# fgnt/pb_bss

Measured on AMD Instinct MI355X. Metric: cACGMM EM iterations/sec on F=513,T=500,D=8,K=3, higher is better.
Workload: dtype f64; 1 GPU; BASELINE configs[1]: 8-mic 3-source cACGMM, F=513 T=500 D=8 K=3, complex64 STFT resident in HBM, fit_predict; utterances=1

## Files before the change

pb_bss_amd/csrc/cacgmm_em.hpp:

```cpp
#pragma once
#include "pbbss.h"
#include "wave_la.hpp"
#include "embed_dev.hpp"

namespace pbbss {

struct EmArgs {
  const void* y;
  int64_t B;
  int T;
  const double* gamma0;
  const double* q0;
  const double* in_eigvec;
  const double* in_eigval;
  const double* in_weight;
  int64_t wb, wk, wt;
  const double* saliency;
  const uint8_t* activity;
  const uint8_t* final_activity;
  double* out_eigvec;
  double* out_eigval;
  double* out_weight;
  int32_t* out_status;
  double* out_aff;
  double* out_q;
  double* out_logpdf;
  double* out_cov;
  char* scratch;
  size_t scratch_stride;
  unsigned long long* prof;
  int T_total;
  int split_groups;
  int split_window;
  int64_t b_first;
  double* xslab;
  unsigned* xcount;
  int* xerror;
  int xepoch;
  int split_prio;
  int main_grid;
  unsigned lds_given;
  unsigned xbuf_given;
  unsigned spin_limit;
  int wgroup;
  double* gsum;
  double* gaff;
  double* gw;
  unsigned* gcount;
  double* out_weight_shared;
  int iterations;
  int covariance_norm;
  int weight_mode;
  int layout;
  int final_predict;
  int force_eig;
  double aff_eps;
  double final_eps;
  double eig_floor;
};

struct JointExtras {
  const double* extra_logpdf;
  double spatial_weight;
  const int* perm;
  const double* state_in;
  double* state_out;
  int emit_model;
  double* weight_fk_out;
  int main_grid;
  unsigned lds_given;
  unsigned xbuf_given;
};

struct JointMs {
  int mode;
  double* q_out;
  double* lndet_out;
  double* weight_fk_out;
  unsigned lds_given;
  int main_grid;
  SpectralFin fin;
};

template <int D, int K, typename YS, bool SPILL = false>
struct EmKernel {
  static constexpr int DP = (D + 1) / 2;
  static constexpr int NOFF = D * (D - 1) / 2;
  static constexpr int NA = D * D;
  static constexpr int NDW = (D + kEmWaves - 1) / kEmWaves;
  static constexpr int NOW = (NOFF + kEmWaves - 1) / kEmWaves;
#ifndef PBBSS_E_CHUNK
#define PBBSS_E_CHUNK 1
#endif
#ifndef PBBSS_E_PAIR
#define PBBSS_E_PAIR 0
#endif
#ifndef PBBSS_M_PREFETCH
#define PBBSS_M_PREFETCH 0
#endif
  static constexpr int kOperandChunk = PBBSS_E_CHUNK;
  using YS4 = typename std::conditional<std::is_same<YS, float>::value, float4, double4>::type;
  using YS2 = typename std::conditional<std::is_same<YS, float>::value, float2, double2>::type;

  struct Lds {
    YS* ybuf;
    double* inv_n2;
    double* wbuf;
    double* cpack;
    double* apack;
    double* wgt;
    double* detm;
    double* rdet;
    double* red;
    double* ssum;
    int* dete;
    int* status;
    int* flags;
    unsigned short* wbtab;
    double* sink;
    int Tp;
  };

  static constexpr int kFC = 64;
  static __host__ __device__ __forceinline__ int padded_frames(int T) { return (T + kFC - 1) & ~(kFC - 1); }
  static __host__ __device__ __forceinline__ int yoff(int dp, int t) {
    return ((((t >> 6) * DP + dp) << 6) + (t & 63)) * 4;
  }
  static __host__ __device__ __forceinline__ int woff(int k, int t) {
    return (((t >> 6) * K + k) << 6) + (t & 63);
  }
  static __host__ __device__ size_t frame_bytes(int T) {
    size_t Tp = (size_t)padded_frames(T);
    return (size_t)DP * Tp * 4 * sizeof(YS) + Tp * 8 + (size_t)K * Tp * 8;
  }
  static __host__ __device__ size_t small_bytes() {
    size_t n = 0;
    n += (size_t)K * NA * 8;
    n += (size_t)K * NA * 8;
    n += (size_t)K * 8 * 4;
    n += (size_t)kEmWaves * K * 8;
    n += (size_t)K * 4 * 2 + 16;
    n += wbtab_bytes() + 8;
    return n;
  }
  static __host__ __device__ size_t lds_bytes(int T) {
    size_t n = small_bytes() + (SPILL ? 0 : frame_bytes(T));
    return (n + 15) & ~(size_t)15;
  }
  static __host__ __device__ size_t scratch_bytes(int T) {
    return SPILL ? ((frame_bytes(T) + 255) & ~(size_t)255) : 0;
  }

  static __device__ Lds carve_small(char* p, int Tp) {
    Lds L;
    L.Tp = Tp;
    L.ybuf = nullptr;
    L.inv_n2 = nullptr;
    L.wbuf = nullptr;
    carve_small_into(L, p);
    return L;
  }

  static __device__ Lds carve(char* base, int T, char* scratch = nullptr) {
    Lds L;
    L.Tp = padded_frames(T);
    char* p = base;
    char* f = SPILL ? scratch : base;
    L.ybuf = reinterpret_cast<YS*>(f);
    f += (size_t)DP * L.Tp * 4 * sizeof(YS);
    L.inv_n2 = reinterpret_cast<double*>(f);
    f += (size_t)L.Tp * 8;
    L.wbuf = reinterpret_cast<double*>(f);
    f += (size_t)K * L.Tp * 8;
    if (!SPILL) p = f;
    carve_small_into(L, p);
    fill_wbtab(L);
    return L;
  }

  static __device__ __forceinline__ void carve_small_into(Lds& L, char* p) {
    L.cpack = reinterpret_cast<double*>(p);
    p += (size_t)K * NA * 8;
    L.apack = reinterpret_cast<double*>(p);
    p += (size_t)K * NA * 8;
    L.wgt = reinterpret_cast<double*>(p);
    p += K * 8;
    L.detm = reinterpret_cast<double*>(p);
    p += K * 8;
    L.rdet = reinterpret_cast<double*>(p);
    p += K * 8;
    L.ssum = reinterpret_cast<double*>(p);
    p += K * 8;
    L.red = reinterpret_cast<double*>(p);
    p += kEmWaves * K * 8;
    L.dete = reinterpret_cast<int*>(p);
    p += K * 4;
    L.status = reinterpret_cast<int*>(p);
    p += K * 4;
    L.flags = reinterpret_cast<int*>(p);
    p += 16;
    L.wbtab = reinterpret_cast<unsigned short*>(p);
    p += wbtab_bytes();
    L.sink = reinterpret_cast<double*>(p);
  }

  static __device__ __forceinline__ int t_stride(const EmArgs& a) {
    return a.T_total ? a.T_total : a.T;
  }

  static __device__ __forceinline__ void load_frame(const Lds& L, int t, double (&re)[D],
                                                    double (&im)[D]) {
    PBBSS_DEV_ASSERT(t >= 0 && t < L.Tp);
    static_for<0, DP>([&](auto dpc) {
      constexpr int dp = dpc;
      YS4 v = *reinterpret_cast<const YS4*>(L.ybuf + yoff(dp, t));
      re[2 * dp] = (double)v.x;
      im[2 * dp] = (double)v.y;
      if constexpr (2 * dp + 1 < D) {
        re[2 * dp + 1] = (double)v.z;
        im[2 * dp + 1] = (double)v.w;
      }
    });
  }

  static __device__ void phase_load(const EmArgs& a, const Lds& L, int64_t b, int tid,
                                    int tf = 0) {
    const int T = a.T;
    const int TS = t_stride(a);
    const YS2* yg = reinterpret_cast<const YS2*>(a.y);
    bool zero_seen = false;
    for (int t = tid; t < L.Tp; t += kEmThreads) {
      double n2 = 0.0;
      YS vr[2 * DP], vi[2 * DP];
#pragma unroll
      for (int d = 0; d < 2 * DP; ++d) {
        vr[d] = (YS)0;
        vi[d] = (YS)0;
      }
      if (t < T) {
#pragma unroll
        for (int d = 0; d < D; ++d) {
          size_t idx = (a.layout == PBBSS_LAYOUT_TD) ? ((size_t)b * TS + tf + t) * D + d
                                                     : ((size_t)b * D + d) * TS + tf + t;
          YS2 v = yg[idx];
          vr[d] = v.x;
          vi[d] = v.y;
          n2 += (double)v.x * (double)v.x + (double)v.y * (double)v.y;
        }
      }
#pragma unroll
      for (int dp = 0; dp < DP; ++dp) {
        YS4 o;
        o.x = vr[2 * dp];
        o.y = vi[2 * dp];
        o.z = vr[2 * dp + 1];
        o.w = vi[2 * dp + 1];
        *reinterpret_cast<YS4*>(L.ybuf + yoff(dp, t)) = o;
      }
      double inv;
      if (a.layout == PBBSS_LAYOUT_TD) {
        inv = (n2 > 0.0) ? 1.0 / n2 : 0.0;
      } else {
        inv = 1.0;
      }
      L.inv_n2[t] = (t < T) ? inv : 0.0;
      if (t < T && !(n2 > 0.0)) zero_seen = true;
      if (t >= T) {
#pragma unroll
        for (int k = 0; k < K; ++k) L.wbuf[woff(k, t)] = 0.0;
      }
    }
    if (zero_seen) atomicOr(L.flags, 1);
  }

  static __device__ __forceinline__ double mweight(double g_sal, double q, double inv_n2) {
    return g_sal / fmax(q, 10.0 * kTiny) * inv_n2;
  }

  static __device__ void phase_init_gamma(const EmArgs& a, const Lds& L, int64_t b, int tid,
                                          int wave, int lane, int tf = 0) {
    const int TS = t_stride(a);
    double s[K];
#pragma unroll
    for (int k = 0; k < K; ++k) s[k] = 0.0;
    for (int t = tid; t < a.T; t += kEmThreads) {
      double sal = a.saliency ? a.saliency[(size_t)b * TS + tf + t] : 1.0;
      double inv = L.inv_n2[t];
#pragma unroll
      for (int k = 0; k < K; ++k) {
        size_t idx = ((size_t)b * K + k) * TS + tf + t;
        double g = a.gamma0[idx] * sal;
        double q = a.q0 ? a.q0[idx] : 1.0;
        L.wbuf[woff(k, t)] = mweight(g, q, inv);
        if (a.gaff && a.weight_mode == PBBSS_WEIGHT_SHARED_KT)
          __hip_atomic_store(a.gaff + idx, g, __ATOMIC_RELAXED, __HIP_MEMORY_SCOPE_AGENT);
        s[k] += g;
      }
    }
#pragma unroll
    for (int k = 0; k < K; ++k) {
      double tot = wave_sum(s[k]);
      if (lane == 0) L.red[wave * K + k] = tot;
    }
  }

  template <bool FINAL, bool TW, bool JOINT = false, bool PAIR = false, bool PERM = false>
  static __device__ void phase_e(const EmArgs& a, const Lds& L, int64_t b, int tid, int wave,
                                 int lane, double eps, int tf = 0,
                                 const JointExtras* jx = nullptr,
                                 const double* w_kt = nullptr,
                                 double* pub_kt = nullptr) {
    tid = opaque(tid);
    lane = opaque(lane);
    const int TS = t_stride(a);
    static_assert(!JOINT || !PAIR, "joint E-step is written for one frame per lane");
    double s[K];
#pragma unroll
    for (int k = 0; k < K; ++k) s[k] = 0.0;
    double jlogdet[K];
#pragma unroll
    for (int k = 0; k < K; ++k)
      jlogdet[k] = JOINT ? log(L.detm[k]) + (double)L.dete[k] * 0.6931471805599453 : 0.0;
    auto pass = [&](int t0, auto nfc) {
      constexpr int NF = decltype(nfc)::value;
      if (t0 + wave * kWave >= padded_frames(a.T)) return;
      int tl[NF];
      int tt[NF];
      bool ok[NF];
      bool inl[NF];
      double re[NF][D], im[NF][D], q[NF][K];
#pragma unroll
      for (int f = 0; f < NF; ++f) {
        int t = t0 + f * kEmThreads + tid;
        ok[f] = t < a.T;
        inl[f] = (f == 0) || t < padded_frames(a.T);
        tt[f] = ok[f] ? t : (a.T - 1);
        tl[f] = (f == 0) ? t : min(t, padded_frames(a.T) - 1);
        load_frame(L, tl[f], re[f], im[f]);
#pragma unroll
        for (int k = 0; k < K; ++k) q[f][k] = 0.0;
      }
      {
        constexpr int NG = (NA + 15) / 16;
        double areg[K][NG];
#pragma unroll
        for (int k = 0; k < K; ++k) {
#pragma unroll
          for (int g = 0; g < NG; ++g) {
            const int e = 16 * g + (lane & 15);
            areg[k][g] = L.apack[k * NA + (e < NA ? e : NA - 1)];
          }
        }
        static_for<0, D>([&](auto ic) {
// ... 128 lines not shown
          double qq = fmax(fabs(q[f][k] * inv), kTiny);
          q[f][k] = qq;
          int e;
          double m = frexp(qq, &e);
          double rm = fast_rcp(m);
          rq[k] = ldexp(rm, -e);
          val[k] = rdet[k] * ipow<D>(rm);
          ex[k] = -(e * D + dete[k]);
          emax = max(emax, ex[k]);
        }
        double g[K], den = 0.0;
#pragma unroll
        for (int k = 0; k < K; ++k) {
          double w;
          if constexpr (TW) {
            w = w_kt ? __hip_atomic_load(w_kt + (size_t)k * TS + tf + t, __ATOMIC_RELAXED,
                                         __HIP_MEMORY_SCOPE_AGENT)
                     : a.in_weight[b * a.wb + k * a.wk + (int64_t)(tf + t) * a.wt];
          } else {
            w = wgt[k];
          }
          double v = ldexp(val[k], ex[k] - emax) * w;
          const uint8_t* act = FINAL ? a.final_activity : a.activity;
          if (act) v *= (double)act[((size_t)b * K + k) * TS + tf + t];
          g[k] = v;
          den += v;
        }
        const double poison = den - den;
        den = fmax(den, kTiny);
        const double rden = fast_rcp(den);
        const double sal = (!FINAL && a.saliency) ? a.saliency[(size_t)b * TS + tf + t] : 1.0;
        const double invp = inv + poison;
#pragma unroll
        for (int k = 0; k < K; ++k) {
          double gam = g[k] * rden;
          if (!FINAL || eps != 0.0) gam = fmin(fmax(gam, eps), 1.0 - eps);
          if constexpr (FINAL) {
            gam += poison;
            if (ok[f]) {
              size_t idx = ((size_t)b * K + k) * TS + tf + t;
              if (a.out_aff) a.out_aff[idx] = gam;
              if (a.out_q) a.out_q[idx] = q[f][k];
              if (a.out_logpdf) {
                a.out_logpdf[idx] = -(double)D * log(q[f][k]) -
                                    (log(detm[k]) + (double)dete[k] * 0.6931471805599453);
              }
            }
          } else {
            double gs = ok[f] ? gam * sal : 0.0;
            if (pub_kt && ok[f])
              __hip_atomic_store(pub_kt + (size_t)k * TS + tf + t, gs, __ATOMIC_RELAXED,
                                 __HIP_MEMORY_SCOPE_AGENT);
            double rqk = fmin(rq[k], 1.0 / (10.0 * kTiny));
            if (f == 0 || inl[f]) L.wbuf[woff(k, tl[f])] = gs * rqk * invp;
            s[k] += gs;
          }
        }
      }
      }
    };
    {
      int t0 = 0;
      if constexpr (PAIR) {
        for (; a.T - t0 > kEmThreads; t0 += 2 * kEmThreads) pass(t0, std::integral_constant<int, 2>{});
      }
      for (; t0 < a.T; t0 += kEmThreads) pass(t0, std::integral_constant<int, 1>{});
    }
    if constexpr (!FINAL) wave_class_sums<K>(s, lane, L.red + wave * K);
  }

  static constexpr int NSLOT = NDW + 2 * NOW;
  static constexpr int NACC = ((K * NSLOT + 15) / 16) * 16;

  struct EntryMap {
    int dwave[D], drank[D];
    int pwave[NOFF > 0 ? NOFF : 1], prank[NOFF > 0 ? NOFF : 1];
    unsigned long long dcode[kEmWaves], pcode[kEmWaves];
  };
  static constexpr EntryMap make_entry_map() {
    EntryMap m{};
    int nd[kEmWaves] = {}, np[kEmWaves] = {};
    for (int w = 0; w < kEmWaves; ++w) {
      m.dcode[w] = ~0ull;
      m.pcode[w] = ~0ull;
    }
    for (int i = 0; i < D; ++i) {
      int w = i % kEmWaves;
      if (D == 8) w = (i < 2) ? 0 : (i < 4) ? 3 : (i < 6) ? 1 : 2;
      m.dwave[i] = w;
      m.drank[i] = nd[w]++;
    }
    for (int p = 0; p < NOFF; ++p) {
      const int i = tri_i<D>(p), j = tri_j<D>(p);
      int w = p % kEmWaves;
      if (D == 8) {
        if (j < 4) w = 0;
        else if (i >= 4) w = 1;
        else if (i == 0 && j == 4) w = 0;
        else if (i == 3 && j == 7) w = 1;
        else w = (i < 2) ? 2 : 3;
      }
      m.pwave[p] = w;
      m.prank[p] = np[w]++;
    }
    for (int i = 0; i < D; ++i) {
      const int w = m.dwave[i], r = m.drank[i];
      m.dcode[w] = (m.dcode[w] & ~(15ull << (4 * r))) | ((unsigned long long)i << (4 * r));
    }
    for (int p = 0; p < NOFF; ++p) {
      const int w = m.pwave[p], r = m.prank[p];
      m.pcode[w] = (m.pcode[w] & ~(31ull << (5 * r))) | ((unsigned long long)p << (5 * r));
    }
    return m;
  }
  static constexpr EntryMap kMap = make_entry_map();
  static constexpr bool entry_map_fits() {
    for (int i = 0; i < D; ++i)
      if (kMap.drank[i] >= NDW) return false;
    for (int p = 0; p < NOFF; ++p)
      if (kMap.prank[p] >= NOW) return false;
    return true;
  }
  static_assert(entry_map_fits(), "a wave owns more entries than it has accumulator slots");

  static constexpr int kWbR = NACC / 16;
  static __host__ __device__ constexpr size_t wbtab_bytes() {
    return ((size_t)kEmWaves * 16 * kWbR * sizeof(unsigned short) + 7) & ~(size_t)7;
  }
  template <bool ROUND_ROBIN = false>
  static __device__ __forceinline__ void fill_wbtab(const Lds& L) {
    const int tid = threadIdx.x;
    if (tid >= kEmWaves * 16) return;
    const int w = tid >> 4, g = tid & 15;
    const unsigned long long dcode = kMap.dcode[w], pcode = kMap.pcode[w];
    const int sink = (int)(L.sink - L.cpack);
#pragma unroll
    for (int m = 0; m < kWbR; ++m) {
      const int idx = kWbR * g + m;
      int off = sink;
      if (idx < K * NSLOT) {
        const int k = idx / NSLOT, sl = idx % NSLOT;
        const bool dg = sl < NDW;
        const int u = ROUND_ROBIN
                          ? (dg ? sl * kEmWaves + w : ((sl - NDW) >> 1) * kEmWaves + w)
                          : (dg ? (int)((dcode >> (4 * sl)) & 15)
                                : (int)((pcode >> (5 * ((sl - NDW) >> 1))) & 31));
        const int e = dg ? u : D + 2 * u + ((sl - NDW) & 1);
        if (u < (dg ? D : NOFF)) off = k * NA + e;
      }
      L.wbtab[(w * 16 + g) * kWbR + m] = (unsigned short)off;
    }
  }

  template <int W>
  static __device__ void phase_m(const EmArgs& a, const Lds& L, int lane, int c_begin = 0,
                                 int c_end = -1, double* cpack_out = nullptr) {
    lane = opaque(lane);
    double acc[NACC];
    const YS* yp = L.ybuf + (size_t)lane * 4 + (size_t)c_begin * (DP * kFC * 4);
    const double* wp = L.wbuf + lane + (size_t)c_begin * (K * kFC);
    struct Raw {
      YS4 v[DP];
      double w[K];
    };
    auto fetch = [&](Raw& r) {
      static_for<0, DP>([&](auto dpc) {
        constexpr int dp = dpc;
        r.v[dp] = *reinterpret_cast<const YS4*>(yp + dp * (kFC * 4));
      });
#pragma unroll
      for (int k = 0; k < K; ++k) r.w[k] = wp[k * kFC];
      yp += DP * kFC * 4;
      wp += K * kFC;
    };
    auto compute = [&](const Raw& r, auto firstc) {
      constexpr bool FIRST = firstc;
      double re[D], im[D];
      static_for<0, DP>([&](auto dpc) {
        constexpr int dp = dpc;
        re[2 * dp] = (double)r.v[dp].x;
        im[2 * dp] = (double)r.v[dp].y;
        if constexpr (2 * dp + 1 < D) {
          re[2 * dp + 1] = (double)r.v[dp].z;
          im[2 * dp + 1] = (double)r.v[dp].w;
        }
      });
      const double (&w)[K] = r.w;
      static_for<0, D>([&](auto ic) {
        constexpr int i = ic;
        if constexpr (kMap.dwave[i] == W) {
          double dg = re[i] * re[i] + im[i] * im[i];
#pragma unroll
          for (int k = 0; k < K; ++k) {
            double& x = acc[k * NSLOT + kMap.drank[i]];
            x = FIRST ? w[k] * dg : fma(w[k], dg, x);
          }
        }
      });
      static_for<0, NOFF>([&](auto pc) {
        constexpr int p = pc;
        if constexpr (kMap.pwave[p] == W) {
          constexpr int i = tri_i<D>(p), j = tri_j<D>(p);
          constexpr int s = NDW + 2 * kMap.prank[p];
          double pr = re[i] * re[j] + im[i] * im[j];
          double pim = im[i] * re[j] - re[i] * im[j];
#pragma unroll
          for (int k = 0; k < K; ++k) {
            double& xr = acc[k * NSLOT + s];
            double& xi = acc[k * NSLOT + s + 1];
            xr = FIRST ? w[k] * pr : fma(w[k], pr, xr);
            xi = FIRST ? w[k] * pim : fma(w[k], pim, xi);
          }
        }
      });
    };
    static_for<0, NACC>([&](auto xc) {
      constexpr int x = xc;
      constexpr int sl = x % NSLOT;
      constexpr bool used =
          x < K * NSLOT &&
          (sl < NDW ? (int)((kMap.dcode[W] >> (4 * sl)) & 15) < D
                    : (int)((kMap.pcode[W] >> (5 * ((sl - NDW) >> 1))) & 31) < NOFF);
      if constexpr (!used) acc[x] = 0.0;
    });
    const int nchunk = (c_end < 0 ? (padded_frames(a.T) >> 6) : c_end) - c_begin;
#if PBBSS_M_PREFETCH
    {
      Raw A, B;
      fetch(A);
      if (nchunk > 1) {
        fetch(B);
        __builtin_amdgcn_sched_barrier(0);
        compute(A, std::true_type{});
        int c = nchunk - 1;
        while (c > 2) {
          fetch(A);
          __builtin_amdgcn_sched_barrier(0);
          compute(B, std::false_type{});
          fetch(B);
          __builtin_amdgcn_sched_barrier(0);
          compute(A, std::false_type{});
          c -= 2;
        }
        if (c == 2) {
          fetch(A);
          __builtin_amdgcn_sched_barrier(0);
          compute(B, std::false_type{});
          compute(A, std::false_type{});
        } else {
          compute(B, std::false_type{});
        }
      } else {
        compute(A, std::true_type{});
      }
    }
#else
    {
      Raw r;
      fetch(r);
      compute(r, std::true_type{});
      for (int c = nchunk; c > 1; --c) {
        fetch(r);
        compute(r, std::false_type{});
      }
    }
#endif
#ifdef PBBSS_PHASE_PROFILE
    unsigned long long tm0 = __builtin_readcyclecounter(), tm1 = tm0;
#endif
    if (a.split_groups == 0) __builtin_amdgcn_s_setprio(1);
    wave_reduce_scatter<NACC>(acc, lane);
#ifdef PBBSS_PHASE_PROFILE
    tm1 = __builtin_readcyclecounter();
#endif
    if ((lane & 3) == 0) {
      const unsigned short* tab = L.wbtab + (W * 16 + ((lane >> 2) & 15)) * kWbR;
      double* dst = cpack_out ? cpack_out : L.cpack;
#pragma unroll
      for (int m = 0; m < kWbR; ++m) dst[tab[m]] = acc[m];
    }
    if (a.split_groups == 0) __builtin_amdgcn_s_setprio(0);
#ifdef PBBSS_PHASE_PROFILE
    if (a.prof && lane == 0 && W == 0) {
      unsigned long long tm2 = __builtin_readcyclecounter();
      atomicAdd(a.prof + 64, tm1 - tm0);
      atomicAdd(a.prof + 65, tm2 - tm1);
      atomicAdd(a.prof + 66, 1ull);
    }
#endif
  }

  static __device__ __forceinline__ int pair_index(int i, int j) {
    return i * D - (i * (i + 1)) / 2 + (j - i - 1);
  }

  static __device__ __forceinline__ void cov_entry(const Lds& L, int k, int i, int j, double& re,
                                                   double& im) {
    if (i == j) {
      re = L.cpack[k * NA + i];
      im = 0.0;
    } else {
      const int lo = min(i, j), hi = max(i, j);
      const double2 v = *reinterpret_cast<const double2*>(L.cpack + k * NA + D + 2 * pair_index(lo, hi));
      re = v.x;
      im = (i < j) ? v.y : -v.y;
    }
  }

  static __device__ __forceinline__ void store_apack(const Lds& L, int k, LaneIJ c, double gre,
                                                     double gim) {
    if (c.i < D && c.j < D) {
      if (c.i == c.j) {
        L.apack[k * NA + c.i] = gre;
      } else if (c.i < c.j) {
        int p = pair_index(c.i, c.j);
        L.apack[k * NA + D + 2 * p] = 2.0 * gre;
        L.apack[k * NA + D + 2 * p + 1] = 2.0 * gim;
      }
    }
  }

  static __device__ __forceinline__ void inverse_from_eig(double vre, double vim, double lam_col,
                                                          LaneIJ c, double& gre, double& gim) {
    gre = 0.0;
    gim = 0.0;
#pragma unroll
    for (int e = 0; e < D; ++e) {
      double il = 1.0 / lane_get(lam_col, ij_lane(0, e));
      double ar = lane_get(vre, ij_lane(c.i, e)), ai = lane_get(vim, ij_lane(c.i, e));
      double br = lane_get(vre, ij_lane(c.j, e)), bi = lane_get(vim, ij_lane(c.j, e));
      gre += (ar * br + ai * bi) * il;
      gim += (ai * br - ar * bi) * il;
    }
  }

  static __device__ void factor_class(const EmArgs& a, const Lds& L, int64_t b, int k, int lane,
                                      bool last) {
    if (a.split_groups == 0) __builtin_amdgcn_s_setprio(3);
    lane = opaque(lane);
    const LaneIJ c = lane_ij(lane);
    const bool valid = c.i < D && c.j < D;
#ifdef PBBSS_PHASE_PROFILE
    unsigned long long fs[6] = {0, 0, 0, 0, 0, 0};
    int fsn = 0;
#define PBBSS_FSTAMP fs[fsn++] = __builtin_readcyclecounter();
    PBBSS_FSTAMP
#else
#define PBBSS_FSTAMP
#endif
    double are = 0.0, aim = 0.0;
    if (valid) cov_entry(L, k, c.i, c.j, are, aim);
    double S = 0.0, tot = 0.0;
#pragma unroll
    for (int kk = 0; kk < K; ++kk) {
      double sk = 0.0;
#pragma unroll
      for (int w = 0; w < kEmWaves; ++w) sk += L.red[w * K + kk];
      tot += fabs(sk);
      S = (kk == k) ? sk : S;
    }
    const double scale = (double)D * fast_rcp(fmax(S, kTiny));
    are *= scale;
    aim *= scale;
    int st = 0;
    if (last && a.out_cov && valid) {
      double* oc = a.out_cov + ((((size_t)b * K + k) * D + c.i) * D + c.j) * 2;
      oc[0] = are;
      oc[1] = aim;
    }
    bool need_eig = last || a.force_eig || (*L.flags & 1);
    PBBSS_FSTAMP
    if (!need_eig) {
      double gre = are, gim = aim;
      ScaledReal det;
      double trc = wave_sum((valid && c.i == c.j) ? are : 0.0);
      int info = wave_hpd_inverse<D>(gre, gim, c, det);
      bool ok = (info == 0);
      PBBSS_FSTAMP
      if (ok) {
        store_apack(L, k, c, gre, gim);
        if (lane == 0) {
          L.detm[k] = det.m;
          L.rdet[k] = fast_rcp(det.m);
          L.dete[k] = det.e;
        }
        double fro2 = wave_sum(valid ? gre * gre + gim * gim : 0.0);
        const double bound2 = trc * trc * fro2;
        ok = isfinite(bound2) && (bound2 * (a.eig_floor * a.eig_floor) < 1e-4) && (bound2 < 1e26);
      }
      if (!ok) {
        need_eig = true;
        st |= PBBSS_ST_SLOWPATH;
      }
      PBBSS_FSTAMP
#ifdef PBBSS_PHASE_PROFILE
      if (a.prof && lane == 0 && k == 0 && !need_eig) {
        atomicAdd(a.prof + 67, fs[1] - fs[0]);
        atomicAdd(a.prof + 68, fs[2] - fs[1]);
        atomicAdd(a.prof + 69, fs[3] - fs[2]);
        atomicAdd(a.prof + 70, 1ull);
      }
#endif
    }
    if (need_eig) {
      const bool finite_in = isfinite(are) && isfinite(aim);
      if (wave_or(finite_in ? 0 : 1)) st |= PBBSS_ST_NONFINITE;
    }
    if (need_eig) {
      if (a.covariance_norm == PBBSS_COVNORM_TRACE) {
        double tr = wave_sum((valid && c.i == c.j) ? are : 0.0);
        double it = 1.0 / fmax(tr, kTiny);
        are *= it;
        aim *= it;
      }
      double vre, vim;
      int sweeps = wave_jacobi_heev<D>(are, aim, c, vre, vim);
      if (sweeps < 0) st |= PBBSS_ST_EIG_NOCONV;
      double lam = lane_get(are, ij_lane(c.j, c.j));
      double lmax = wave_max((c.i == 0 && c.j < D) ? lam : -1.79e308);
      double lout;
      if (a.covariance_norm == PBBSS_COVNORM_EIGENVALUE) {
        lout = lam / fmax(lmax, kTiny);
        if (lout < a.eig_floor) {
          lout = a.eig_floor;
          if (c.i == 0 && c.j < D) st |= PBBSS_ST_FLOORED;
        }
      } else {
        double fl = lmax * a.eig_floor;
        lout = lam;
        if (lout < fl) {
          lout = fl;
          if (c.i == 0 && c.j < D) st |= PBBSS_ST_FLOORED;
        }
      }
      if (c.i == 0 && c.j < D && !isfinite(lout)) st |= PBBSS_ST_NONFINITE;
      st = wave_or(st);
      if (c.j >= D) lout = 1.0;
      if (last) {
        int rank = wave_sort_rank<D>(lam, c);
        if (valid) {
          if (a.out_eigvec) {
            double* ov = a.out_eigvec + ((((size_t)b * K + k) * D + c.i) * D + rank) * 2;
            ov[0] = vre;
            ov[1] = vim;
          }
          if (a.out_eigval && c.i == 0) a.out_eigval[((size_t)b * K + k) * D + rank] = lout;
        }
      }
      double gre, gim;
      inverse_from_eig(vre, vim, lout, c, gre, gim);
      store_apack(L, k, c, gre, gim);
      ScaledReal det{1.0, 0};
#pragma unroll
      for (int e = 0; e < D; ++e) scaled_mul(det, fmax(lane_get(lout, ij_lane(0, e)), kTiny));
      if (lane == 0) {
        L.detm[k] = det.m;
        L.rdet[k] = 1.0 / det.m;
        L.dete[k] = det.e;
      }
    }
    if (lane == 0) {
      L.status[k] |= st;
      double wnew;
      if (a.weight_mode >= PBBSS_WEIGHT_SHARED_K) {
        wnew = L.wgt[k];
      } else if (a.weight_mode == PBBSS_WEIGHT_UNIFORM) {
        wnew = 1.0 / K;
      } else if (a.saliency) {
        wnew = S / ((tot == 0.0) ? 1e-10 : tot);
      } else {
        wnew = S / (double)t_stride(a);
      }
      L.wgt[k] = wnew;
    }
    if (a.split_groups == 0) __builtin_amdgcn_s_setprio(0);
  }

  static __device__ void prep_from_model(const EmArgs& a, const Lds& L, int64_t b, int k,
                                         int lane) {
    const LaneIJ c = lane_ij(lane);
    const bool valid = c.i < D && c.j < D;
    double vre = 0.0, vim = 0.0, lam = 1.0;
    if (valid) {
      const double* v = a.in_eigvec + ((((size_t)b * K + k) * D + c.i) * D + c.j) * 2;
      vre = v[0];
      vim = v[1];
      lam = a.in_eigval[((size_t)b * K + k) * D + c.j];
    }
    double gre, gim;
    inverse_from_eig(vre, vim, lam, c, gre, gim);
    store_apack(L, k, c, gre, gim);
    ScaledReal det{1.0, 0};
#pragma unroll
    for (int e = 0; e < D; ++e) scaled_mul(det, fmax(lane_get(lam, ij_lane(0, e)), kTiny));
    if (lane == 0) {
      L.detm[k] = det.m;
      L.rdet[k] = 1.0 / det.m;
      L.dete[k] = det.e;
      L.wgt[k] = a.in_weight ? a.in_weight[b * a.wb + k * a.wk] : 1.0 / K;
    }
  }

  static __device__ __forceinline__ void quad_forms(const Lds& L, int t, double (&q)[K]) {
    double re[D], im[D];
    load_frame(L, t, re, im);
#pragma unroll
    for (int k = 0; k < K; ++k) q[k] = 0.0;
    static_for<0, D>([&](auto ic) {
      constexpr int i = ic;
      double dg = re[i] * re[i] + im[i] * im[i];
#pragma unroll
      for (int k = 0; k < K; ++k) q[k] = fma(L.apack[k * NA + i], dg, q[k]);
    });
    static_for<0, NOFF>([&](auto pc) {
      constexpr int p = pc;
      constexpr int i = tri_i<D>(p), j = tri_j<D>(p);
      double pr = re[i] * re[j] + im[i] * im[j];
      double pim = im[i] * re[j] - re[i] * im[j];
#pragma unroll
      for (int k = 0; k < K; ++k)
        q[k] = fma(L.apack[k * NA + D + 2 * p], pr, fma(L.apack[k * NA + D + 2 * p + 1], pim, q[k]));
    });
    const double inv = L.inv_n2[t];
#pragma unroll
    for (int k = 0; k < K; ++k) q[k] = fmax(fabs(q[k] * inv), kTiny);
  }

  static __device__ __forceinline__ void quad_forms_pipelined(const Lds& L, const double (&re)[D],
                                                              const double (&im)[D],
                                                              double (&q)[K]) {
    constexpr int NCH = (NOFF + kOperandChunk - 1) / kOperandChunk;
    double op[2][kOperandChunk][K][2];
    auto fetch = [&](auto cc, auto bb) {
      constexpr int c = cc, bsel = bb;
#pragma unroll
      for (int x = 0; x < kOperandChunk; ++x) {
        if (c * kOperandChunk + x < NOFF) {
#pragma unroll
          for (int k = 0; k < K; ++k) {
            op[bsel][x][k][0] = L.apack[k * NA + D + 2 * (c * kOperandChunk + x)];
            op[bsel][x][k][1] = L.apack[k * NA + D + 2 * (c * kOperandChunk + x) + 1];
          }
        }
      }
    };
#pragma unroll
    for (int k = 0; k < K; ++k) q[k] = 0.0;
    if constexpr (NCH > 0) fetch(std::integral_constant<int, 0>{}, std::integral_constant<int, 0>{});
    asm volatile("" ::: "memory");
    static_for<0, D>([&](auto ic) {
      constexpr int i = ic;
      double ad[K];
#pragma unroll
      for (int k = 0; k < K; ++k) ad[k] = L.apack[k * NA + i];
      double dg = re[i] * re[i] + im[i] * im[i];
#pragma unroll
      for (int k = 0; k < K; ++k) q[k] = fma(ad[k], dg, q[k]);
    });
    static_for<0, NCH>([&](auto cc) {
      constexpr int c = cc;
      constexpr int cur = c & 1;
      if constexpr (c + 1 < NCH) {
        fetch(std::integral_constant<int, c + 1>{}, std::integral_constant<int, 1 - cur>{});
      }
      asm volatile("" ::: "memory");
      __builtin_amdgcn_sched_barrier(0);
      static_for<0, kOperandChunk>([&](auto xc) {
        constexpr int x = xc;
        constexpr int p = c * kOperandChunk + x;
        if constexpr (p < NOFF) {
          constexpr int i = tri_i<D>(p), j = tri_j<D>(p);
          double pr = re[i] * re[j] + im[i] * im[j];
          double pim = im[i] * re[j] - re[i] * im[j];
#pragma unroll
          for (int k = 0; k < K; ++k)
            q[k] = fma(op[cur][x][k][0], pr, fma(op[cur][x][k][1], pim, q[k]));
        }
      });
#pragma unroll
      for (int k = 0; k < K; ++k) asm volatile("" : "+v"(q[k])::"memory");
      __builtin_amdgcn_sched_barrier(0);
    });
  }

  static __device__ __forceinline__ void nth_permutation(int p, int (&perm)[K]) {
    int fact = 1;
#pragma unroll
    for (int i = 2; i < K; ++i) fact *= i;
    unsigned used = 0;
#pragma unroll
    for (int i = 0; i < K; ++i) {
      int d = p / fact;
      p -= d * fact;
      if (i < K - 1) fact /= (K - 1 - i);
      int pick = 0;
#pragma unroll
      for (int c = 0, seen = 0; c < K; ++c) {
        if (!(used >> c & 1)) {
          if (seen == d) pick = c;
          ++seen;
        }
      }
      used |= 1u << pick;
      perm[i] = pick;
    }
  }

  static __device__ void phase_joint_pa(const EmArgs& a, const Lds& L, int64_t b, int tid,
                                        int wave, int lane, const JointExtras& jx, int* perm_out) {
    for (int t = tid; t < a.T; t += kEmThreads) {
      double q[K];
      quad_forms(L, t, q);
#pragma unroll
      for (int k = 0; k < K; ++k) {
// ... 815 lines not shown
          tk[k] = 0.0;
#pragma unroll
          for (int w = 0; w < kEmWaves; ++w) tk[k] += tmp[(w * K + k) * kSliceFrames + tid];
          norm += fabs(tk[k]);
        }
#pragma unroll
        for (int k = 0; k < K; ++k) {
          const double w = a.saliency ? tk[k] / ((norm == 0.0) ? 1e-10 : norm)
                                      : tk[k] / (double)a.wgroup;
          __hip_atomic_store(dst + (size_t)k * TS + t, w, __ATOMIC_RELAXED,
                             __HIP_MEMORY_SCOPE_AGENT);
        }
        asm volatile("s_waitcnt vmcnt(0)" ::: "memory");
      }
      __syncthreads();
      if (tid == 0)
        __hip_atomic_fetch_add(a.gcount + grp * 16 + 8, 1u, __ATOMIC_RELAXED,
                               __HIP_MEMORY_SCOPE_AGENT);
    }
  }

  static __device__ const double* shared_acquire_kt(const EmArgs& a, int64_t b, int step, int tid) {
    const int TS = t_stride(a);
    const int64_t grp = b / a.wgroup;
    const int nsl = (TS + kSliceFrames - 1) / kSliceFrames;
    if (tid == 0) shared_spin(a, a.gcount + grp * 16 + 8, (unsigned)nsl * (unsigned)(step + 1));
    __syncthreads();
    return a.gw + ((size_t)(step & 1) * (a.B / a.wgroup) + grp) * K * TS;
  }

  static __device__ void run_shared(const EmArgs& a, char* smem) {
    const int tid = threadIdx.x;
    const int wave = __builtin_amdgcn_readfirstlane(tid >> 6);
    const int lane = tid & 63;
    const Lds L = carve(smem, a.T, nullptr);
    const int64_t b = a.b_first + blockIdx.x;
    const bool kt = (a.weight_mode == PBBSS_WEIGHT_SHARED_KT);
    const int TS = t_stride(a);
    if (tid < K) L.status[tid] = 0;
    if (tid == 0) *L.flags = 0;
    __syncthreads();
    phase_load(a, L, b, tid);
    __syncthreads();
    const bool model_in = (a.gamma0 == nullptr);
    if (model_in) {
      for (int k = wave; k < K; k += kEmWaves) prep_from_model(a, L, b, k, lane);
      __syncthreads();
      if (!kt && tid < K) L.wgt[tid] = a.in_weight[(b / a.wgroup) * K + tid];
    } else {
      phase_init_gamma(a, L, b, tid, wave, lane);
    }
    if (kt) asm volatile("s_waitcnt vmcnt(0)" ::: "memory");
    __syncthreads();
    for (int it = 0; it < a.iterations; ++it) {
      if (it > 0 || model_in) {
        double* pub = kt ? a.gaff + ((size_t)(it & 1) * a.B + b) * K * TS : nullptr;
        if (kt) {
          const double* w_kt = (it == 0) ? a.in_weight + (b / a.wgroup) * (int64_t)K * TS
                                         : shared_acquire_kt(a, b, it - 1, tid);
          phase_e<false, true, false, false>(a, L, b, tid, wave, lane, a.aff_eps, 0, nullptr, w_kt,
                                             pub);
        } else {
          if (it > 0) shared_acquire_k(a, L, b, it - 1, tid, wave, lane);
          phase_e<false, false, false, PBBSS_E_PAIR != 0>(a, L, b, tid, wave, lane, a.aff_eps);
        }
        if (kt) asm volatile("s_waitcnt vmcnt(0)" ::: "memory");
        __syncthreads();
      }
      shared_post(a, L, b, it, tid);
      switch (wave) {
        case 0: phase_m<0>(a, L, lane); break;
        case 1: phase_m<1>(a, L, lane); break;
        case 2: phase_m<2>(a, L, lane); break;
        default: phase_m<3>(a, L, lane); break;
      }
      __syncthreads();
      const bool last = (it == a.iterations - 1);
      for (int k = wave; k < K; k += kEmWaves) factor_class(a, L, b, k, lane, last);
      __syncthreads();
      if (kt) shared_reduce_kt(a, L, b, it, tid, wave, lane);
    }
    const double* w_kt = nullptr;
    if (a.iterations > 0) {
      const int64_t grp = b / a.wgroup;
      if (kt) {
        w_kt = shared_acquire_kt(a, b, a.iterations - 1, tid);
        if (a.out_weight_shared && b == grp * a.wgroup) {
          for (int i = tid; i < K * TS; i += kEmThreads)
            a.out_weight_shared[(size_t)grp * K * TS + i] =
                __hip_atomic_load(w_kt + i, __ATOMIC_RELAXED, __HIP_MEMORY_SCOPE_AGENT);
        }
      } else {
        shared_acquire_k(a, L, b, a.iterations - 1, tid, wave, lane);
        if (a.out_weight_shared && b == grp * a.wgroup && tid < K)
          a.out_weight_shared[(size_t)grp * K + tid] = L.wgt[tid];
      }
    }
    if (tid < K && a.out_status) {
      int st = L.status[tid];
      if (split_failed(a))
        st |= PBBSS_ST_EIG_NOCONV | PBBSS_ST_NONFINITE;
      a.out_status[(size_t)b * K + tid] = st;
    }
    if (a.final_predict) {
      if (w_kt) {
        phase_e<true, true>(a, L, b, tid, wave, lane, a.final_eps, 0, nullptr, w_kt);
      } else {
        phase_e<true, false>(a, L, b, tid, wave, lane, a.final_eps);
      }
    }
  }

  static __device__ void run(const EmArgs& a, char* smem) {
    const int tid = threadIdx.x;
    const int wave = __builtin_amdgcn_readfirstlane(tid >> 6);
    const int lane = tid & 63;
    PBBSS_DEV_ASSERT(a.lds_given == 0 || lds_bytes(a.T) <= a.lds_given);
    const Lds L = carve(smem, a.T, SPILL ? a.scratch + (size_t)blockIdx.x * a.scratch_stride : nullptr);
#ifdef PBBSS_PHASE_PROFILE
    unsigned long long pc[8] = {0, 0, 0, 0, 0, 0, 0, 0};
    unsigned long long tprev = __builtin_readcyclecounter();
#define PBBSS_TICK(i)                                        \
  {                                                          \
    unsigned long long tn = __builtin_readcyclecounter();    \
    pc[i] += tn - tprev;                                     \
    tprev = tn;                                              \
  }
#else
#define PBBSS_TICK(i)
#endif
    for (int64_t b = blockIdx.x; b < a.B; b += gridDim.x) {
      __syncthreads();
      if (tid < K) L.status[tid] = 0;
      if (tid == 0) *L.flags = 0;
      __syncthreads();
      phase_load(a, L, b, tid);
      __syncthreads();
      const bool model_in = (a.gamma0 == nullptr);
      if (model_in) {
        for (int k = wave; k < K; k += kEmWaves) prep_from_model(a, L, b, k, lane);
      } else {
        phase_init_gamma(a, L, b, tid, wave, lane);
      }
      __syncthreads();
      PBBSS_TICK(0)
      for (int it = 0; it < a.iterations; ++it) {
        if (it > 0 || model_in) {
          phase_e<false, false, false, PBBSS_E_PAIR != 0>(a, L, b, tid, wave, lane, a.aff_eps);
          PBBSS_TICK(1)
          __syncthreads();
          PBBSS_TICK(2)
        }
        switch (wave) {
          case 0: phase_m<0>(a, L, lane); break;
          case 1: phase_m<1>(a, L, lane); break;
          case 2: phase_m<2>(a, L, lane); break;
          default: phase_m<3>(a, L, lane); break;
        }
        PBBSS_TICK(3)
        __syncthreads();
        PBBSS_TICK(4)
        const bool last = (it == a.iterations - 1);
        for (int k = wave; k < K; k += kEmWaves) factor_class(a, L, b, k, lane, last);
        PBBSS_TICK(5)
        __syncthreads();
        PBBSS_TICK(6)
      }
      if (tid < K) {
        if (a.out_weight && a.iterations > 0) a.out_weight[(size_t)b * K + tid] = L.wgt[tid];
        if (a.out_status) a.out_status[(size_t)b * K + tid] = L.status[tid];
      }
      if (a.final_predict) {
        if (a.iterations == 0 && a.wt != 0) {
          phase_e<true, true>(a, L, b, tid, wave, lane, a.final_eps);
        } else {
          phase_e<true, false>(a, L, b, tid, wave, lane, a.final_eps);
        }
      }
      PBBSS_TICK(7)
    }
#ifdef PBBSS_PHASE_PROFILE
    if (a.prof && lane == 0) {
      for (int i = 0; i < 8; ++i) atomicAdd(a.prof + wave * 8 + i, pc[i]);
    }
#endif
  }
};

#ifndef PBBSS_EM_WAVES
#define PBBSS_EM_WAVES 3
#endif
constexpr int em_waves_per_simd(int K) { return K <= 4 ? PBBSS_EM_WAVES : 2; }

template <int D, int K, typename YS, bool SPILL>
__global__ void __launch_bounds__(kEmThreads, em_waves_per_simd(K)) cacgmm_em_kernel(EmArgs a) {
  extern __shared__ __attribute__((aligned(16))) char smem[];
  EmKernel<D, K, YS, SPILL>::run(a, smem);
}


template <int D, int K, typename YS, bool PA>
__global__ void __launch_bounds__(kEmThreads, em_waves_per_simd(K))
    cacgmm_joint_kernel(EmArgs a, JointExtras jx) {
  extern __shared__ __attribute__((aligned(16))) char smem[];
  EmKernel<D, K, YS, false>::template run_joint<PA>(a, jx, smem);
}

template <int D, int K, typename YS, int MODE>
__global__ void __launch_bounds__(kEmThreads, em_waves_per_simd(K))
    cacgmm_joint_ms_kernel(EmArgs a, JointMs jm) {
  extern __shared__ __attribute__((aligned(16))) char smem[];
  EmKernel<D, K, YS, false>::template run_joint_ms<MODE>(a, jm, smem);
}

template <int D, int K, typename YS>
__global__ void __launch_bounds__(kEmThreads, em_waves_per_simd(K)) cacgmm_em_shared_kernel(EmArgs a) {
  extern __shared__ __attribute__((aligned(16))) char smem[];
  EmKernel<D, K, YS, false>::run_shared(a, smem);
}

template <int D, int K, typename YS>
__global__ void __launch_bounds__(kEmThreads, em_waves_per_simd(K)) cacgmm_em_split_kernel(EmArgs a) {
  extern __shared__ __attribute__((aligned(16))) char smem[];
  EmKernel<D, K, YS, false>::run_split(a, smem, (int)blockIdx.x, (int)gridDim.x);
}

}
```

Before: 79580 EM iterations/s (utterance-iterations, whole job).

## Hoist class scale and weight prep into M-step, table-drive factor loads/stores

Moves the per-class reduction of E-step sums (scale and new mixture weight) out of factor_class and into phase_m, computing it after the first chunk so it overlaps with the accumulation loop. An inline-asm pin keeps the compiler from sinking it. It also adds an LDS lookup table mapping each lane to its packed covariance offset and conjugation/store flags, replacing the per-lane index arithmetic in cov_entry and store_apack. This trims serial work on the critical factor path between barriers, at the cost of extra LDS, register pressure in phase_m, and duplicated logic.

```diff
diff --git a/pb_bss_amd/csrc/cacgmm_em.hpp b/pb_bss_amd/csrc/cacgmm_em.hpp
--- a/pb_bss_amd/csrc/cacgmm_em.hpp
+++ b/pb_bss_amd/csrc/cacgmm_em.hpp
@@ -112,10 +112,12 @@
     double* detm;
     double* rdet;
     double* red;
+    double* scale;
     double* ssum;
     int* dete;
     int* status;
     int* flags;
+    unsigned* ftab;
     unsigned short* wbtab;
     double* sink;
     int Tp;
@@ -139,7 +141,9 @@
     n += (size_t)K * NA * 8;
     n += (size_t)K * 8 * 4;
     n += (size_t)kEmWaves * K * 8;
+    n += (size_t)K * 8;
     n += (size_t)K * 4 * 2 + 16;
+    n += (size_t)kWave * 4;
     n += wbtab_bytes() + 8;
     return n;
   }
@@ -175,6 +179,7 @@
     if (!SPILL) p = f;
     carve_small_into(L, p);
     fill_wbtab(L);
+    fill_ftab(L);
     return L;
   }
 
@@ -193,12 +198,16 @@
     p += K * 8;
     L.red = reinterpret_cast<double*>(p);
     p += kEmWaves * K * 8;
+    L.scale = reinterpret_cast<double*>(p);
+    p += K * 8;
     L.dete = reinterpret_cast<int*>(p);
     p += K * 4;
     L.status = reinterpret_cast<int*>(p);
     p += K * 4;
     L.flags = reinterpret_cast<int*>(p);
     p += 16;
+    L.ftab = reinterpret_cast<unsigned*>(p);
+    p += kWave * 4;
     L.wbtab = reinterpret_cast<unsigned short*>(p);
     p += wbtab_bytes();
     L.sink = reinterpret_cast<double*>(p);
@@ -633,10 +642,67 @@
     }
   }
 
-  template <int W>
+  static constexpr unsigned kFtDiag = 1u << 10, kFtConj = 1u << 11, kFtValid = 1u << 12;
+  static constexpr unsigned kFtStore = 1u << 26, kFtStoreDiag = 1u << 27;
+  static __device__ __forceinline__ void fill_ftab(const Lds& L) {
+    const int tid = threadIdx.x;
+    if (tid >= kWave) return;
+    const LaneIJ c = lane_ij(tid);
+    unsigned t = 0;
+    if (c.i < D && c.j < D) {
+      if (c.i == c.j) {
+        t = (unsigned)(c.i * 8) | kFtDiag | kFtValid | ((unsigned)(c.i * 8) << 16) | kFtStore |
+            kFtStoreDiag;
+      } else {
+        const int lo = min(c.i, c.j), hi = max(c.i, c.j);
+        const unsigned off = (unsigned)(D + 2 * pair_index(lo, hi)) * 8;
+        t = off | kFtValid;
+        if (c.i < c.j) t |= (off << 16) | kFtStore;
+        else t |= kFtConj;
+      }
+    }
+    L.ftab[tid] = t;
+  }
+
+  static __device__ __forceinline__ void pinned(double& x, const double* after) {
+    asm volatile(""
+                 : "+v"(x)
+                 : "v"(after[0]), "v"(after[1]), "v"(after[2]), "v"(after[3]), "v"(after[4]),
+                   "v"(after[5]), "v"(after[6]), "v"(after[7]), "v"(after[8]), "v"(after[9]),
+                   "v"(after[10]), "v"(after[11]), "v"(after[12]), "v"(after[13]), "v"(after[14]),
+                   "v"(after[15]));
+  }
+  static __device__ __forceinline__ void class_prep(const EmArgs& a, const double (&red)[kEmWaves * K],
+                                                    int k, const double (&after)[48], double& scale,
+                                                    double& wnew) {
+    double S = 0.0, tot = 0.0;
+#pragma unroll
+    for (int kk = 0; kk < K; ++kk) {
+      double sk = 0.0;
+#pragma unroll
+      for (int w = 0; w < kEmWaves; ++w) sk += red[w * K + kk];
+      tot += fabs(sk);
+      S = (kk == k) ? sk : S;
+    }
+    scale = (double)D * fast_rcp(fmax(S, kTiny));
+    pinned(scale, after);
+    pinned(tot, after + 16);
+    const double den = a.saliency ? ((tot == 0.0) ? 1e-10 : tot) : (double)t_stride(a);
+    wnew = S / den;
+    pinned(wnew, after + 32);
+    if (a.weight_mode == PBBSS_WEIGHT_UNIFORM) wnew = 1.0 / K;
+  }
+
+  template <int W, bool PREP = false>
   static __device__ void phase_m(const EmArgs& a, const Lds& L, int lane, int c_begin = 0,
                                  int c_end = -1, double* cpack_out = nullptr) {
     lane = opaque(lane);
+    constexpr bool kPrep = PREP && W < K;
+    double red[kEmWaves * K];
+    if constexpr (kPrep) {
+#pragma unroll
+      for (int i = 0; i < kEmWaves * K; ++i) red[i] = L.red[i];
+    }
     double acc[NACC];
     const YS* yp = L.ybuf + (size_t)lane * 4 + (size_t)c_begin * (DP * kFC * 4);
     const double* wp = L.wbuf + lane + (size_t)c_begin * (K * kFC);
@@ -704,6 +770,25 @@
                     : (int)((kMap.pcode[W] >> (5 * ((sl - NDW) >> 1))) & 31) < NOFF);
       if constexpr (!used) acc[x] = 0.0;
     });
+    auto prep = [&]() {
+      if constexpr (kPrep) {
+        constexpr int kOwn = (K - W + kEmWaves - 1) / kEmWaves;
+        double scale[kOwn], wnew[kOwn];
+        double after[48];
+#pragma unroll
+        for (int i = 0; i < 48; ++i) after[i] = acc[i < K * NSLOT ? i : K * NSLOT - 1];
+#pragma unroll
+        for (int n = 0; n < kOwn; ++n)
+          class_prep(a, red, W + n * kEmWaves, after, scale[n], wnew[n]);
+        if (lane == 0) {
+#pragma unroll
+          for (int n = 0; n < kOwn; ++n) {
+            L.scale[W + n * kEmWaves] = scale[n];
+            if (a.weight_mode < PBBSS_WEIGHT_SHARED_K) L.wgt[W + n * kEmWaves] = wnew[n];
+          }
+        }
+      }
+    };
     const int nchunk = (c_end < 0 ? (padded_frames(a.T) >> 6) : c_end) - c_begin;
 #if PBBSS_M_PREFETCH
     {
@@ -713,6 +798,7 @@
         fetch(B);
         __builtin_amdgcn_sched_barrier(0);
         compute(A, std::true_type{});
+        prep();
         int c = nchunk - 1;
         while (c > 2) {
           fetch(A);
@@ -733,6 +819,7 @@
         }
       } else {
         compute(A, std::true_type{});
+        prep();
       }
     }
 #else
@@ -740,6 +827,7 @@
       Raw r;
       fetch(r);
       compute(r, std::true_type{});
+      prep();
       for (int c = nchunk; c > 1; --c) {
         fetch(r);
         compute(r, std::false_type{});
@@ -801,6 +889,17 @@
     }
   }
 
+  static __device__ __forceinline__ void store_apack_tab(const Lds& L, int k, unsigned ft,
+                                                         double gre, double gim) {
+    if (ft & kFtStore) {
+      double* dst = reinterpret_cast<double*>(reinterpret_cast<char*>(L.apack + k * NA) +
+                                              ((ft >> 16) & 0x3FFu));
+      const bool dg = (ft & kFtStoreDiag) != 0;
+      dst[0] = dg ? gre : 2.0 * gre;
+      if (!dg) dst[1] = 2.0 * gim;
+    }
+  }
+
   static __device__ __forceinline__ void inverse_from_eig(double vre, double vim, double lam_col,
                                                           LaneIJ c, double& gre, double& gim) {
     gre = 0.0;
@@ -815,6 +914,7 @@
     }
   }
 
+  template <bool HOISTED = false>
   static __device__ void factor_class(const EmArgs& a, const Lds& L, int64_t b, int k, int lane,
                                       bool last) {
     if (a.split_groups == 0) __builtin_amdgcn_s_setprio(3);
@@ -830,17 +930,28 @@
 #define PBBSS_FSTAMP
 #endif
     double are = 0.0, aim = 0.0;
-    if (valid) cov_entry(L, k, c.i, c.j, are, aim);
-    double S = 0.0, tot = 0.0;
-#pragma unroll
-    for (int kk = 0; kk < K; ++kk) {
-      double sk = 0.0;
-#pragma unroll
-      for (int w = 0; w < kEmWaves; ++w) sk += L.red[w * K + kk];
-      tot += fabs(sk);
-      S = (kk == k) ? sk : S;
-    }
-    const double scale = (double)D * fast_rcp(fmax(S, kTiny));
+    double S = 0.0, tot = 0.0, scale;
+    unsigned ft = 0;
+    if constexpr (HOISTED) {
+      ft = L.ftab[lane];
+      const double* cp = reinterpret_cast<const double*>(
+          reinterpret_cast<const char*>(L.cpack + k * NA) + (ft & 0x3FFu));
+      const double v0 = cp[0], v1 = cp[1];
+      scale = L.scale[k];
+      are = (ft & kFtValid) ? v0 : 0.0;
+      aim = (ft & kFtDiag) || !(ft & kFtValid) ? 0.0 : ((ft & kFtConj) ? -v1 : v1);
+    } else {
+      if (valid) cov_entry(L, k, c.i, c.j, are, aim);
+#pragma unroll
+      for (int kk = 0; kk < K; ++kk) {
+        double sk = 0.0;
+#pragma unroll
+        for (int w = 0; w < kEmWaves; ++w) sk += L.red[w * K + kk];
+        tot += fabs(sk);
+        S = (kk == k) ? sk : S;
+      }
+      scale = (double)D * fast_rcp(fmax(S, kTiny));
+    }
     are *= scale;
     aim *= scale;
     int st = 0;
@@ -859,11 +970,21 @@
       bool ok = (info == 0);
       PBBSS_FSTAMP
       if (ok) {
-        store_apack(L, k, c, gre, gim);
-        if (lane == 0) {
-          L.detm[k] = det.m;
-          L.rdet[k] = fast_rcp(det.m);
-          L.dete[k] = det.e;
+        if constexpr (HOISTED) {
+          const double rdet = fast_rcp(det.m);
+          store_apack_tab(L, k, ft, gre, gim);
+          if (lane == 0) {
+            L.detm[k] = det.m;
+            L.rdet[k] = rdet;
+            L.dete[k] = det.e;
+          }
+        } else {
+          store_apack(L, k, c, gre, gim);
+          if (lane == 0) {
+            L.detm[k] = det.m;
+            L.rdet[k] = fast_rcp(det.m);
+            L.dete[k] = det.e;
+          }
         }
         double fro2 = wave_sum(valid ? gre * gre + gim * gim : 0.0);
         const double bound2 = trc * trc * fro2;
@@ -930,7 +1051,8 @@
       }
       double gre, gim;
       inverse_from_eig(vre, vim, lout, c, gre, gim);
-      store_apack(L, k, c, gre, gim);
+      if constexpr (HOISTED) store_apack_tab(L, k, ft, gre, gim);
+      else store_apack(L, k, c, gre, gim);
       ScaledReal det{1.0, 0};
 #pragma unroll
       for (int e = 0; e < D; ++e) scaled_mul(det, fmax(lane_get(lout, ij_lane(0, e)), kTiny));
@@ -940,7 +1062,9 @@
         L.dete[k] = det.e;
       }
     }
-    if (lane == 0) {
+    if constexpr (HOISTED) {
+      if (lane == 0) L.status[k] |= st;
+    } else if (lane == 0) {
       L.status[k] |= st;
       double wnew;
       if (a.weight_mode >= PBBSS_WEIGHT_SHARED_K) {
@@ -2062,16 +2186,16 @@
           PBBSS_TICK(2)
         }
         switch (wave) {
-          case 0: phase_m<0>(a, L, lane); break;
-          case 1: phase_m<1>(a, L, lane); break;
-          case 2: phase_m<2>(a, L, lane); break;
-          default: phase_m<3>(a, L, lane); break;
+          case 0: phase_m<0, true>(a, L, lane); break;
+          case 1: phase_m<1, true>(a, L, lane); break;
+          case 2: phase_m<2, true>(a, L, lane); break;
+          default: phase_m<3, true>(a, L, lane); break;
         }
         PBBSS_TICK(3)
         __syncthreads();
         PBBSS_TICK(4)
         const bool last = (it == a.iterations - 1);
-        for (int k = wave; k < K; k += kEmWaves) factor_class(a, L, b, k, lane, last);
+        for (int k = wave; k < K; k += kEmWaves) factor_class<true>(a, L, b, k, lane, last);
         PBBSS_TICK(5)
         __syncthreads();
         PBBSS_TICK(6)
```

Result: no change. 80350 EM iterations/s (utterance-iterations, whole job) (median of 6 runs) (+1.0%).
